# sdrobert/pydrobert-speech

Measured on AMD Instinct MI355X. Metric: frames/s (whole node) + HBM-roofline %, 40-mel fbank 16kHz 25/10ms, higher is better.
Workload: dtype f32

## Files before the change

pydrobert-speech_amd/csrc/pds_internal.h:

```cpp
#pragma once
#include <hip/hip_runtime.h>
#include <stdint.h>

#include <exception>
#include <new>
#include <string>

#include "../../include/pds_amd.h"

namespace pds {

void set_error(const std::string &msg);
int32_t hip_fail(hipError_t err, const char *what);

#define PDS_HIP(call)                                       \
  do {                                                      \
    hipError_t _e = (call);                                 \
    if (_e != hipSuccess) return pds::hip_fail(_e, #call);  \
  } while (0)

struct FastTables {
  int kind = 0;
  int n1 = 0, n2 = 0;
  int rows = 0;
  int num_cus = 0;
  float *d_window = nullptr;
  float *d_twiddle = nullptr;
  float *d_tw_special = nullptr;
  float *d_win_half = nullptr;
// ... 1 lines not shown
  float *d_ell_w = nullptr;
  int32_t *d_ell_meta = nullptr;
  int32_t *d_ell_len = nullptr;
  int32_t *d_ell_woff = nullptr;
  int ell_wfloats = 0, ell_slots = 0;
  float *d_seg_w = nullptr;
  int32_t *d_seg_meta = nullptr;
  int seg_rounds = 0, seg_len = 0, seg_wfloats = 0, seg_meta_ints = 0;
  float *d_rs_w = nullptr;
  int32_t *d_rs_meta = nullptr;
  int rs_rounds = 0, rs_len = 0, rs_wfloats = 0;
  float *d_rsn_w = nullptr;
  int32_t *d_rsn_meta = nullptr;
  int rsn_rounds = 0, rsn_len = 0, rsn_wfloats = 0;
  int rs_eslot = -1;
  float *d_ms_w = nullptr;
  int32_t *d_ms_meta = nullptr;
  int ms_rounds = 0, ms_len = 0, ms_wfloats = 0, ms_meta_ints = 0, ms_slots = 0;
  long ms_reads = 0;
  int walk = 0;
  long rs_reads = 0, rs_cost = 0, ell_reads = 0, seg_reads = 0;
  float *d_mf_tab = nullptr;
  int mf_rows = 0;
};

}

struct pds_stft_plan {
  pds_stft_desc d;
  int device = 0;
  int num_bins = 0;
  float *d_window_f32 = nullptr;
  double *d_window_f64 = nullptr;
  int32_t *d_row_ptr = nullptr;
  int32_t *d_col = nullptr;
  float *d_val_f32 = nullptr;
  double *d_val_f64 = nullptr;
  float2 *d_tw_f32 = nullptr;
  double2 *d_tw_f64 = nullptr;
  pds::FastTables fast;
};

namespace pds {
struct SiFftTables {
  int blocks = 0;
  bool big = false;
// ... 126 lines not shown
```

pydrobert-speech_amd/csrc/stft_fast.hip:

```cpp
#include "stft_wave_launch.h"

namespace pds {

#if PDS_STAMPS
unsigned long long *g_stamp_buf = nullptr;
extern "C" __attribute__((visibility("default"))) void pds_debug_set_stamp_buffer(unsigned long long *d_buf) {
  g_stamp_buf = d_buf;
}
#endif

extern "C" __attribute__((visibility("default"))) int32_t pds_build_experiments(void) { return PDS_EXPERIMENTS ? 1 : 0; }

bool fast_has_f64in(const pds_stft_plan *plan) { return plan->fast.kind && fast_f64in_kind(plan->fast.kind); }

static int fast_geometry_rows(const FastTables &ft, int *minw);

bool fast_has_fused_cmvn(const pds_stft_plan *plan) {
  const FastTables &ft = plan->fast;
  int minw = 0;
  if (!ft.kind || ft.n2 != 16 || (ft.n1 != 32 && ft.n1 != 64) || !fast_geometry_rows(ft, &minw)) return false;
  return ft.walk == 1 || ft.walk == 3 || (ft.walk == 2 && minw <= 2);
}

bool fast_has_fused_deltas(const pds_stft_plan *plan) {
  const FastTables &ft = plan->fast;
  return ft.kind && fast_deltas_kind(ft.kind) && ft.rsn_rounds >= 1 && ft.rsn_rounds <= 2 &&
         (!plan->d.include_energy || ft.rs_eslot >= 0);
}

__global__ __launch_bounds__(1024) void chunk_prefix_kernel(const int64_t *nframes, int B, int groups, int64_t *prefix) {
  __shared__ int64_t part[1024];
  const int per = (B + 1023) / 1024, lo = threadIdx.x * per, hi = lo + per < B ? lo + per : B;
  int64_t sum = 0;
  for (int b = lo; b < hi; ++b) sum += (nframes[b] + groups - 1) / groups;
// ... 168 lines not shown
    }
    ell_len[sl] = longest;
    ell_woff[sl] = (int32_t)ell_w.size();
    const int wstride = longest + 4;
    ell_w.resize(ell_w.size() + (size_t)n2 * wstride, 0.0f);
    for (int j = 0; j < n2; ++j) {
      const int f = sl * n2 + j < d.num_filts ? order[sl * n2 + j] : -1;
      if (first[j] + longest > pstr)
        first[j] = (pstr - longest) & ~3;
      if (first[j] < 0) return PDS_OK;
      ell_meta[(size_t)sl * n2 + j] = first[j] | ((f + 1) << 16);
      if (f < 0) continue;
      for (int q = row_ptr[f]; q < row_ptr[f + 1]; ++q) {
        const int t = col[q] - first[j];
        if (t < 0 || t >= longest) return PDS_OK;
        ell_w[(size_t)ell_woff[sl] + (size_t)j * wstride + t] = (float)val[q];
      }
    }
  }
  if (ell_w.empty()) ell_w.assign(4, 0.0f);
  ft.ell_wfloats = (int)ell_w.size();
  ft.ell_slots = slots;
  int32_t rc = PDS_OK;
  const int groups = 64 / n2;
  bool dense_bank = false;
  long dense_reads = 0;
  if ((n2 == 16 || (pow2 && n2 >= 32)) && d.num_filts > 0 && d.num_filts <= 65535) {
    long ell_reads = 0;
    for (int sl = 0; sl < slots; ++sl) ell_reads += 2L * (ell_len[sl] / 4);
    ft.ell_reads = ell_reads;
    const int free_slots = (wave_area_floats(n1, n2) - groups * pstr) / groups;
    int best_len = 0, best_rounds = 0;
    long best_reads = 0, any_reads = 0;
    const char *only_len = std::getenv("PDS_SEG_LEN");
    for (int len : {16, 32, 64}) {
      if (only_len && std::atoi(only_len) != len) continue;
      long nseg = 0;
      for (int f = 0; f < d.num_filts; ++f) nseg += (span(f) + len - 1) / len;
      const int rounds = (int)((nseg + 63) / 64);
      if (rounds == 0 || rounds * 64 > 65535) continue;
      int longest = 0;
      for (int f = 0; f < d.num_filts; ++f) longest = std::max(longest, (span(f) + len - 1) / len);
      const long reads = (long)rounds * (len / 4) * (1 + groups) + rounds + (nseg + 63) / 64 + 4 + 4L * ((longest + 3) / 4);
      if (!any_reads || reads < any_reads) any_reads = reads;
      if (rounds * 64 > free_slots) continue;
      if (!best_len || reads < best_reads) best_len = len, best_rounds = rounds, best_reads = reads;
// ... 19 lines not shown
        const int count = (span(f) + len - 1) / len;
        seg_meta[(size_t)nslots + f] = slot | (count << 16);
        const int base = count ? col[row_ptr[f]] & ~3 : 0;
        for (int k = 0; k < count; ++k, ++slot) {
          int first = base + k * len;
          if (first + len > pstr) first = (pstr - len) & ~3;
          if (first < 0) ok = false;
          seg_meta[slot] = first;
          for (int q = row_ptr[f]; q < row_ptr[f + 1]; ++q) {
            if (col[q] < base + k * len || col[q] >= base + (k + 1) * len) continue;
            const int t = col[q] - first;
            if (t < 0 || t >= len) ok = false; else seg_w[(size_t)slot * wstride + t] = (float)val[q];
          }
        }
      }
      if (ok) {
        ft.seg_reads = best_reads;
        ft.seg_rounds = best_rounds;
        ft.seg_len = len;
        ft.seg_wfloats = (int)seg_w.size();
        ft.seg_meta_ints = (int)seg_meta.size();
        if (rc == PDS_OK) rc = upload(&ft.d_seg_w, seg_w.data(), seg_w.size());
        if (rc == PDS_OK) rc = upload(&ft.d_seg_meta, seg_meta.data(), seg_meta.size());
      }
    }
  }
  if (n2 == 16 && rc == PDS_OK) {
    RsegTables rs;
    const int area_floats = wave_area_floats(n1, n2);
    if (build_rseg(d.num_filts, row_ptr, col, val, N / 2 + 1, area_floats / 4, 8, rs)) {
      ft.rs_rounds = rs.rounds;
      ft.rs_len = rs.seg_len;
      ft.rs_wfloats = (int)rs.w.size();
      ft.rs_reads = rs.reads_per_lane();
      ft.rs_cost = rs.cost;
      RsegTables rn;
      ft.rs_eslot = -1;
      if (rc == PDS_OK && fast_deltas_kind(N) && build_rseg(d.num_filts, row_ptr, col, val, N / 2 + 1, area_floats / 4, 2, rn, true)) {
        ft.rsn_rounds = rn.rounds;
        ft.rsn_len = rn.seg_len;
        ft.rsn_wfloats = (int)rn.w.size();
        for (size_t at = 0; at < rn.meta.size() && ft.rs_eslot < 0; ++at)
          if ((rn.meta[at] >> 16) == 0) ft.rs_eslot = (int)at;
        rc = upload(&ft.d_rsn_w, rn.w.data(), rn.w.size());
        if (rc == PDS_OK) rc = upload(&ft.d_rsn_meta, rn.meta.data(), rn.meta.size());
      }
      if (rc == PDS_OK) rc = upload(&ft.d_rs_w, rs.w.data(), rs.w.size());
      if (rc == PDS_OK) rc = upload(&ft.d_rs_meta, rs.meta.data(), rs.meta.size());
    }
  }
  if (n2 == 16 && pow2 && rc == PDS_OK && dense_bank) {
    MsegTables ms;
    const int area_floats = wave_area_floats(n1, n2);
    const int max_slots = (area_floats - 4 * pstr) / 16;
    if (build_mseg(d.num_filts, row_ptr, col, val, pstr, max_slots, ms)) {
      ft.ms_rounds = ms.rounds;
      ft.ms_slots = ms.slots;
      ft.ms_len = ms.seg_len;
      ft.ms_wfloats = (int)ms.w.size();
      ft.ms_meta_ints = (int)ms.meta.size();
      ft.ms_reads = ms.reads_per_lane();
      rc = upload(&ft.d_ms_w, ms.w.data(), ms.w.size());
      if (rc == PDS_OK) rc = upload(&ft.d_ms_meta, ms.meta.data(), ms.meta.size());
    }
  }
  {
    const char *force = std::getenv("PDS_STFT_WALK");
    ft.walk = ft.seg_rounds > 0 ? 1 : 0;
    const bool ms_stands_in = ft.walk == 0 && dense_bank && ft.ms_rounds > 0 && N >= PDS_MSEG_MIN_N;
    const long other = ft.walk == 1 ? ft.seg_reads : ms_stands_in ? dense_reads : ft.ell_reads;
    if (ft.rs_rounds > 0 && 10 * ft.rs_reads <= 7 * other) ft.walk = 2;
    if (force && std::strcmp(force, "ell") == 0) ft.walk = 0;
    if (force && std::strcmp(force, "seg") == 0) ft.walk = ft.seg_rounds > 0 ? 1 : 0;
    if (force && std::strcmp(force, "rseg") == 0) ft.walk = ft.rs_rounds > 0 ? 2 : ft.walk;
    if ((ft.walk == 1 || (ft.walk == 0 && ms_stands_in)) && ft.ms_rounds > 0 && N >= PDS_MSEG_MIN_N && !force) ft.walk = 3;
    if (force && std::strcmp(force, "mseg") == 0 && ft.ms_rounds > 0) ft.walk = 3;
    if (std::getenv("PDS_DEBUG_PLAN"))
      std::fprintf(stderr,
                   "pds plan N=%d filters=%d: ell slots %d reads %ld | seg rounds %d len %d reads %ld | rseg rounds %d "
                   "len %d reads %ld cost %ld | mseg rounds %d len %d reads %ld -> walk %d\n",
                   N, d.num_filts, ft.ell_slots, ft.ell_reads, ft.seg_rounds, ft.seg_len, ft.seg_reads, ft.rs_rounds,
                   ft.rs_len, ft.rs_reads, ft.rs_cost, ft.ms_rounds, ft.ms_len, ft.ms_reads, ft.walk);
  }
  if (rc == PDS_OK) rc = upload(&ft.d_ell_w, ell_w.data(), ell_w.size());
  if (rc == PDS_OK) rc = upload(&ft.d_ell_meta, ell_meta.data(), ell_meta.size());
  if (rc == PDS_OK) rc = upload(&ft.d_ell_len, ell_len.data(), ell_len.size());
  if (rc == PDS_OK) rc = upload(&ft.d_ell_woff, ell_woff.data(), ell_woff.size());
  if (rc == PDS_OK) rc = upload(&ft.d_window, win.data(), win.size());
  if (rc == PDS_OK) rc = upload(&ft.d_twiddle, tw.data(), tw.size());
  if (((n1 == 32 || n1 == 64) && n2 == 16) || lean_geometry(n1, n2)) {
    std::vector<float> wh(win), seed((size_t)n2 * 6);
    for (float &v : wh) v *= PDS_RDFT_DIT ? 1.0f : 0.5f;
    const int mult[3] = {1, 4, n1 / 4};
    for (int r = 0; r < n2; ++r)
      for (int j = 0; j < 3; ++j) {
        const double ang = -2.0 * M_PI * (double)((r * mult[j]) % N) / (double)N;
        seed[((size_t)r * 3 + j) * 2 + 0] = (float)std::cos(ang);
        seed[((size_t)r * 3 + j) * 2 + 1] = (float)std::sin(ang);
      }
    if (rc == PDS_OK) rc = upload(&ft.d_win_half, wh.data(), wh.size());
    if (rc == PDS_OK) rc = upload(&ft.d_tw_seed, seed.data(), seed.size());
  }
  std::vector<float> tws((size_t)n2 * 2);
  for (int r = 0; r < n2; ++r) {
    const double ang = -2.0 * M_PI * (double)r / (double)(2 * n2);
    tws[2 * r] = (float)std::cos(ang);
    tws[2 * r + 1] = (float)std::sin(ang);
  }
  if (rc == PDS_OK) rc = upload(&ft.d_tw_special, tws.data(), tws.size());
  {
    const char *front = PDS_EXPERIMENTS ? std::getenv("PDS_STFT_FRONT") : nullptr;
    const int rows = (d.frame_length + n2 - 1) / n2;
    int bucket = 0;
    for (int b : {20, 25, 28, 30, 32})
// ... 5 lines not shown
      image.reserve(mt.words());
      image.insert(image.end(), mt.win.begin(), mt.win.end());
      for (int32_t v : mt.off) {
        float f;
        std::memcpy(&f, &v, sizeof f);
        image.push_back(f);
      }
      image.insert(image.end(), mt.emask.begin(), mt.emask.end());
      image.insert(image.end(), mt.a_re.begin(), mt.a_re.end());
      image.insert(image.end(), mt.a_im.begin(), mt.a_im.end());
      image.insert(image.end(), mt.tw.begin(), mt.tw.end());
      rc = upload(&ft.d_mf_tab, image.data(), image.size());
      ft.mf_rows = bucket;
    }
  }
  if (rc != PDS_OK) return rc;
  hipDeviceProp_t prop;
  PDS_HIP(hipGetDeviceProperties(&prop, plan->device));
  ft.num_cus = prop.multiProcessorCount;
  ft.n1 = n1;
  ft.n2 = n2;
  ft.rows = (d.frame_length + n2 - 1) / n2;
  ft.kind = d.dft_size;
  return PDS_OK;
}

void fast_tables_destroy(pds_stft_plan *plan) {
  FastTables &ft = plan->fast;
  (void)hipFree(ft.d_window);
  (void)hipFree(ft.d_twiddle);
  (void)hipFree(ft.d_tw_special);
  (void)hipFree(ft.d_win_half);
  (void)hipFree(ft.d_tw_seed);
  (void)hipFree(ft.d_mf_tab);
  (void)hipFree(ft.d_rs_w);
  (void)hipFree(ft.d_ms_w);
  (void)hipFree(ft.d_ms_meta);
  (void)hipFree(ft.d_rsn_w);
  (void)hipFree(ft.d_rsn_meta);
  (void)hipFree(ft.d_rs_meta);
  (void)hipFree(ft.d_seg_w);
  (void)hipFree(ft.d_seg_meta);
  (void)hipFree(ft.d_ell_w);
  (void)hipFree(ft.d_ell_meta);
  (void)hipFree(ft.d_ell_len);
  (void)hipFree(ft.d_ell_woff);
  ft = FastTables();
}

}
```

pydrobert-speech_amd/csrc/stft_switches.h:

```cpp
#pragma once
namespace pds {

#ifndef PDS_PRIO_PACK
#define PDS_PRIO_PACK 0x103212
#endif
#if PDS_PRIO_PACK == 0xffffff
#define PDS_PHASE(i) __builtin_amdgcn_sched_barrier(0)
#else
#define PDS_PHASE(i) do { if (PDS_PRIO_PACK >= 0) __builtin_amdgcn_s_setprio(((PDS_PRIO_PACK) >> (4 * (i))) & 3); } while (0)
#endif
#ifndef PDS_ABLATE
#define PDS_ABLATE 0
#endif
#ifndef PDS_STAMPS
#define PDS_STAMPS 0
#endif
#if PDS_STAMPS
extern unsigned long long *g_stamp_buf;
#define PDS_STAMP(i, drain)                                               \
  do {                                                                    \
    if (PDS_STAMPS == 2) break;                                           \
    __builtin_amdgcn_sched_barrier(0);                                    \
    if (drain) asm volatile("s_waitcnt vmcnt(0)" ::: "memory");           \
    const unsigned long long now_ = __builtin_readcyclecounter();         \
    st_acc[i] += now_ - st_prev;                                          \
    st_prev = now_;                                                       \
    __builtin_amdgcn_sched_barrier(0);                                    \
  } while (0)
#else
#define PDS_STAMP(i, drain) do { } while (0)
#endif
#ifndef PDS_SEG_DEEP_N
#define PDS_SEG_DEEP_N 1024
#endif
#ifndef PDS_ELL_DEEP_N
#define PDS_ELL_DEEP_N 4096
#endif
#ifndef PDS_MSEG_MIN_N
#define PDS_MSEG_MIN_N 1024
#endif
#ifndef PDS_PAIR_SPLIT
#define PDS_PAIR_SPLIT 1
#endif
#ifndef PDS_N4096_MINW
#define PDS_N4096_MINW 2
#endif
#ifndef PDS_FAST_PROLOGUE
#define PDS_FAST_PROLOGUE 1
#endif
#ifndef PDS_MSEG_RED4
#define PDS_MSEG_RED4 1
#endif
#ifndef PDS_FILTER_UNROLL
#define PDS_FILTER_UNROLL 2
#endif
#ifndef PDS_EXPERIMENTS
#define PDS_EXPERIMENTS 0
#endif
#ifndef PDS_RDFT_DIT
#define PDS_RDFT_DIT (!PDS_EXPERIMENTS)
#endif
#ifndef PDS_WINDOW_CONTRACT
#define PDS_WINDOW_CONTRACT 0
#endif
#ifndef PDS_PACKED_LDS
#define PDS_PACKED_LDS 0
#endif
#ifndef PDS_WALK_DPP_FMAC
#define PDS_WALK_DPP_FMAC 1
#endif
#ifndef PDS_PREEMPH_DPP
// ... 46 lines not shown
```

pydrobert-speech_amd/csrc/stft_wave_kernel.h:

```cpp
#pragma once
#include <algorithm>
#include <atomic>
#include <cmath>
#include <cstdio>
#include <cstdlib>
#include <cstring>
#include <type_traits>
#include <vector>

#include "fft_inlane.h"
#include "mfma_front.h"
#include "rseg_tables.h"
#include "mseg_tables.h"
#include "pds_internal.h"

#include "stft_switches.h"

namespace pds {

__device__ __forceinline__ void keep_alive(float v) { asm volatile("" ::"v"(v)); }

struct FastParams {
  const void *sig;
  const int64_t *offsets, *lengths, *nframes, *row_off;
  void *out;
  int64_t out_stride;
  const float *win_lane;
  const float2 *tw_lane;
  const float2 *tw_special;
  const float *win_half;
  const float2 *tw_seed;
  const float *ell_w;
  const int32_t *ell_meta;
  const int32_t *ell_len;
  const int32_t *ell_woff;
  int ell_wfloats, ell_slots, ell_meta_pad, ell_meta_ints;
  int seg_rounds, seg_len, num_filts;
  int L, S, pad_left, include_energy, use_power, use_log;
  float log_floor, inv_L, preemph;
  double preemph_d;
  int chunks_per_utt, num_utts;
  int waves;
  int area_f;
  unsigned waves_rcp;
  int lds_ticket_off;
  int dyn;
  const float *mf_tab;
  unsigned long long *stamps;
  const int64_t *chunk_prefix;
  double *stat_part;
  int stat_c, stat_cs;
  int lds_stat_off;
// ... 42 lines not shown
}

template <int CTRL>
__device__ __forceinline__ float dpp_add(float x) {
  return x + __int_as_float(__builtin_amdgcn_update_dpp(0, __float_as_int(x), CTRL, 0xf, 0xf, false));
}

__device__ __forceinline__ void wave_sync() {
  __builtin_amdgcn_fence(__ATOMIC_RELEASE, "wavefront");
  __builtin_amdgcn_wave_barrier();
  __builtin_amdgcn_fence(__ATOMIC_ACQUIRE, "wavefront");
}

#ifndef PDS_TWOPASS
#define PDS_TWOPASS 1
#endif
#ifndef PDS_LEAN_2048
#define PDS_LEAN_2048 1
#endif
constexpr bool lean_geometry(int n1, int n2) { return PDS_LEAN_2048 && n1 == 64 && n2 == 32; }
constexpr int wave_area_floats(int n1, int n2) {
  const int cols = (n1 - 1) / 2 + 1, groups = 64 / n2, one_pass = groups * cols * (n2 + 2) * 2;
  return (PDS_TWOPASS && n1 == 64 && n2 == 16) ? 2688 : lean_geometry(n1, n2) ? groups * cols * (n2 + 4) : one_pass;
}
constexpr int win_table_stride(int rows) { return ((rows + 3) & ~3) % 8 == 4 ? ((rows + 3) & ~3) : ((rows + 3) & ~3) + 4; }

template <int N1, int N2, int NROWS>
struct WaveGeom {
  static constexpr int N = N1 * N2;
  static constexpr int NREG = (N1 - 1) / 2;
  static constexpr int COLS = NREG + 1;
  static constexpr int CPL = (COLS + N2 - 1) / N2;
  static constexpr bool FULL = COLS % N2 == 0;
  static constexpr bool DIST = N2 >= 16;
  static constexpr int GROUPS = 64 / N2;
  static constexpr int NB = N / 2 + 1;
  static constexpr int RS = N2 + 2;
  static constexpr bool TWOPASS = PDS_TWOPASS && N1 == 64 && N2 == 16;
  static constexpr bool LEAN = lean_geometry(N1, N2);
  static constexpr int RSF = N2 + 4;
  static constexpr int XROWS = TWOPASS ? N2 : COLS;
  static constexpr int EXCH_F2 = wave_area_floats(N1, N2) / 2;
  static_assert(LEAN ? GROUPS * XROWS * RSF <= EXCH_F2 * 2 : GROUPS * XROWS * RS <= EXCH_F2, "the exchange must fit the wave's area");
  static_assert(!LEAN || (CPL == 1 && N2 >= 32), "lean form: one column per lane");
  static constexpr int PSTR = ((NB + 1 + 15) / 32) * 32 + 16;
  static_assert(GROUPS * PSTR <= EXCH_F2 * 2, "P must fit over the exchange area");
// ... 43 lines not shown
  [[maybe_unused]] const bool stats_on = STATS && p.stat_part != nullptr;
  [[maybe_unused]] auto stat_add4 = [&](const int col, const float (&v)[4], const int nf) {
    double t1 = 0.0, t2 = 0.0;
#pragma unroll
    for (int q = 0; q < 4; ++q)
      if (q < nf) {
        const double d = (double)v[q];
        t1 += d;
        t2 = fma(d, d, t2);
      }
    wstat[col] += t1;
    wstat[p.stat_cs + col] += t2;
  };
  float2 *exch = reinterpret_cast<float2 *>(wbase) + g * G::XROWS * RS;
  [[maybe_unused]] float *xf = wbase + g * (G::XROWS * G::RSF);
  float *Pg = wbase + g * PSTR;
  const int nthreads = p.waves * 64;
  float2 *sw_lds = reinterpret_cast<float2 *>(smem + p.waves * p.area_f);
  int *meta_lds = reinterpret_cast<int *>(sw_lds + N2);
  float *ellw_lds = reinterpret_cast<float *>(meta_lds + p.ell_meta_pad);
  constexpr bool TWCHAIN = (PF && PDS_PF_TW == 1) || (PAIR && (N1 == 32 || N1 == 64)) || (PDS_DLT_CHAIN && DLT > 0 && N1 == 32 && N2 == 16) || G::LEAN ||
                           (N1 == 64 && N2 == 16 && (SEG == 2 || PDS_LEAN_1024));
  constexpr bool WINLDS = PF && PDS_PF_WIN == 1;
  constexpr bool WINUSE = G::LEAN || (N1 == 64 && N2 == 16 && (SEG == 2 || PDS_LEAN_1024));
  constexpr int WSTR = win_table_stride(NROWS);
  [[maybe_unused]] float *win_lds = ellw_lds + (ELL_LDS ? p.ell_wfloats : 0);
  if constexpr (WINLDS || WINUSE) {
    const float *wsrc = TWCHAIN ? p.win_half : p.win_lane;
    for (int i = threadIdx.x; i < N2 * WSTR; i += p.waves * 64) {
      const int rr = i / WSTR, k = i - rr * WSTR;
      win_lds[i] = k < NROWS ? wsrc[rr * N1 + k] : 0.0f;
    }
  }
  if (threadIdx.x < N2) sw_lds[threadIdx.x] = p.tw_special[threadIdx.x];
  constexpr bool DYN = PDS_DYN && !STRETCH && !PF;
  [[maybe_unused]] int *ticket_lds = reinterpret_cast<int *>(smem + p.lds_ticket_off);
  if constexpr (DYN) {
    if (threadIdx.x == 0) *ticket_lds = p.waves;
  }
  if constexpr (STR && G::GROUPS == 4 && (SEG != 0 || (RSG && MINW <= 2))) {
    if (p.stat_part) {
      double *z = reinterpret_cast<double *>(smem + p.lds_stat_off);
      for (int i = threadIdx.x; i < p.waves * 2 * p.stat_cs; i += p.waves * 64) z[i] = 0.0;
    }
  }
  if constexpr (RSG) {
    int4 *rec_lds = reinterpret_cast<int4 *>(meta_lds);
    for (int i = threadIdx.x; i < p.seg_rounds * 64; i += nthreads) {
      const int m = p.ell_meta[i], f = (m >> 16) - 1;
      rec_lds[i] = make_int4((m & 0x3fff) * 16, __float_as_int((m & (1 << 14)) ? 1.0f : 0.0f),
                             __float_as_int((m & (1 << 15)) ? 1.0f : 0.0f),
                             f >= 0 ? ((p.include_energy ? 1 : 0) + f) * (int)sizeof(TOUT) : -1);
    }
  } else {
    for (int i = threadIdx.x; i < p.ell_meta_pad; i += nthreads)
      meta_lds[i] = i < p.ell_meta_ints ? p.ell_meta[i] : 0;
  }
#if PDS_FAST_PROLOGUE
  static_assert((G::EXCH_F2 * 2) % 4 == 0, "wave areas are zeroed 16 bytes at a time");
  if constexpr (ELL_LDS) {
    const float4 *src4 = reinterpret_cast<const float4 *>(p.ell_w);
    float4 *dst4 = reinterpret_cast<float4 *>(ellw_lds);
    for (int i = threadIdx.x; i < (p.ell_wfloats >> 2); i += nthreads) dst4[i] = src4[i];
  }
  {
    float4 *z4 = reinterpret_cast<float4 *>(smem);
    for (int i = threadIdx.x; i < p.waves * (p.area_f / 4); i += nthreads) z4[i] = make_float4(0.0f, 0.0f, 0.0f, 0.0f);
  }
#else
  if constexpr (ELL_LDS)
    for (int i = threadIdx.x; i < p.ell_wfloats; i += nthreads) ellw_lds[i] = p.ell_w[i];
  for (int i = threadIdx.x; i < p.waves * p.area_f; i += nthreads) smem[i] = 0.0f;
#endif
  __syncthreads();

  [[maybe_unused]] float win[(MF || WINLDS || WINUSE) ? 1 : NROWS];
  [[maybe_unused]] float twr[(MF || TWCHAIN) ? 1 : COLS], twi[(MF || TWCHAIN) ? 1 : COLS];
  [[maybe_unused]] float sd[6] = {0.0f, 0.0f, 0.0f, 0.0f, 0.0f, 0.0f};
  [[maybe_unused]] float mwin[MSLOTS], mare[MF + 1], maim[MF + 1], mtwr[4], mtwi[4];
  [[maybe_unused]] unsigned moff[MSLOTS];
  if constexpr (MF > 0) {
    const float *tab = p.mf_tab;
#pragma unroll
    for (int sl = 0; sl < MSLOTS; ++sl) {
      mwin[sl] = tab[sl * 64 + lane];
      moff[sl] = (unsigned)reinterpret_cast<const int *>(tab)[(MSLOTS + sl) * 64 + lane] * 4u;
    }
#pragma unroll
    for (int t = 0; t <= MF; ++t) {
      mare[t] = tab[(3 * MSLOTS + t) * 64 + lane];
      maim[t] = tab[(3 * MSLOTS + MF + 1 + t) * 64 + lane];
    }
#pragma unroll
    for (int v = 0; v < 4; ++v) {
      const float2 t = reinterpret_cast<const float2 *>(tab + (3 * MSLOTS + 2 * (MF + 1)) * 64)[v * 64 + lane];
      mtwr[v] = t.x;
      mtwi[v] = t.y;
    }
  } else {
    if constexpr (!WINLDS && !WINUSE) {
      const float *wsrc = TWCHAIN ? p.win_half : p.win_lane;
#pragma unroll
      for (int n1 = 0; n1 < NROWS; ++n1) win[n1] = wsrc[rho * N1 + n1];
    }
    if constexpr (TWCHAIN) {
#pragma unroll
      for (int j = 0; j < 3; ++j) {
        const float2 t = p.tw_seed[rho * 3 + j];
        sd[2 * j] = t.x;
        sd[2 * j + 1] = t.y;
      }
    } else {
#pragma unroll
      for (int k1 = 1; k1 <= NREG; ++k1) {
        const float2 t = p.tw_lane[rho * COLS + k1];
        twr[k1] = t.x;
        twi[k1] = t.y;
      }
    }
  }
  [[maybe_unused]] float pfv[PF ? NROWS : 1];
  [[maybe_unused]] float wl[WINLDS ? NROWS : 1];
  [[maybe_unused]] auto read_window = [&]() {
    if constexpr (WINLDS) {
      const float4 *w4 = reinterpret_cast<const float4 *>(win_lds + rho * WSTR);
#pragma unroll
      for (int j = 0; j < (NROWS + 3) / 4; ++j) {
        const float4 w = w4[j];
        const float wv[4] = {w.x, w.y, w.z, w.w};
#pragma unroll
        for (int u = 0; u < 4; ++u)
          if (4 * j + u < NROWS) wl[4 * j + u] = wv[u];
      }
    }
  };
  read_window();
  [[maybe_unused]] bool pf_ready = false;
  [[maybe_unused]] const int pf_lane = __mul24(g, p.S) + r;
  const int L = p.L, S = p.S;
  const bool use_power = p.use_power != 0;
  const int col0 = p.include_energy ? 1 : 0;

  int b = 0;
  int wg = blockIdx.x;
#ifndef PDS_NO_XCD_MAP
  if ((gridDim.x & 7) == 0) wg = (wg & 7) * (gridDim.x >> 3) + (wg >> 3);
#endif
  int chunk = wg * p.waves + wave;
  if constexpr (!STRETCH) {
    while (chunk >= p.chunks_per_utt && b < p.num_utts) {
      chunk -= p.chunks_per_utt;
      ++b;
    }
  }
  [[maybe_unused]] int rnd = 0, rb = 0, rc = wg * p.waves;
  if constexpr (DYN) {
    while (rc >= p.chunks_per_utt && rb < p.num_utts) {
      rc -= p.chunks_per_utt;
      ++rb;
// ... 12 lines not shown
    }
    b = rb;
    chunk = rc + o;
    while (chunk >= p.chunks_per_utt && b < p.num_utts) {
      chunk -= p.chunks_per_utt;
      ++b;
    }
  };
  [[maybe_unused]] int ticket_v = 0;
  [[maybe_unused]] auto fetch_ticket = [&]() {
    if (lane == 0) ticket_v = __hip_atomic_fetch_add(ticket_lds, 1, __ATOMIC_RELAXED, __HIP_MEMORY_SCOPE_WORKGROUP);
  };
  [[maybe_unused]] auto next_item_dyn = [&](int &nfr_, int &n_, int64_t &sig_off_, int64_t &out_row_) {
    const int last_b = b;
    take_ticket(__builtin_amdgcn_readfirstlane(ticket_v));
    const int pb_ = b < p.num_utts ? b : last_b;
    nfr_ = (int)load_const(p.nframes + pb_);
    n_ = (int)load_const(p.lengths + pb_);
    sig_off_ = load_const(p.offsets + pb_);
    out_row_ = load_const(p.row_off + pb_);
  };
  int nfr = 0, n = 0;
  int64_t sig_off = 0, out_row = 0;
  if (!STRETCH && b < p.num_utts) {
    nfr = (int)load_const(p.nframes + b);
    n = (int)load_const(p.lengths + b);
    sig_off = load_const(p.offsets + b);
    out_row = load_const(p.row_off + b);
  }
  constexpr int DR = 2;
  [[maybe_unused]] int left = 0, e_lo = 0, e_hi = 0, c_last = -1;
  [[maybe_unused]] bool piece_open = false, ran = false;
  [[maybe_unused]] float Wp[DR][4], Wc[DR][4], e_keep = 0.0f;
  if constexpr (STRETCH) {
    const int gw = wg * p.waves + wave, GW = (int)gridDim.x * p.waves;
    const int total = (int)load_const(p.chunk_prefix + p.num_utts);
    const int per = total / GW, rem = total - per * GW;
    const int pos = gw * per + (gw < rem ? gw : rem);
    left = per + (gw < rem ? 1 : 0);
    int lo = 0, hi = p.num_utts;
    while (left > 0 && hi - lo > 1) {
      const int mid = (lo + hi) >> 1;
      if ((int)load_const(p.chunk_prefix + mid) <= pos) lo = mid; else hi = mid;
    }
    b = lo;
    e_lo = left > 0 ? pos - (int)load_const(p.chunk_prefix + lo) : 0;
    chunk = 0;
#pragma unroll
    for (int rd = 0; rd < DR; ++rd)
#pragma unroll
      for (int q = 0; q < 4; ++q) Wp[rd][q] = Wc[rd][q] = 0.0f;
  }
  [[maybe_unused]] auto emit_rows = [&](const int ce, const float (&nx)[DR][4]) {
    if (p.dl_debug & 2) return;
    const int C = p.dl_inner;
    const int W = (p.dl_order + 1) * C, WS = (W + 3) & ~3;
    float *stage = wbase;
    wave_sync();
#pragma unroll
    for (int rd = 0; rd < DR; ++rd) {
      if (rd >= p.seg_rounds) break;
      const int cb = reinterpret_cast<const int4 *>(meta_lds)[rd * 64 + lane].w;
      const int col = cb >= 0 ? cb >> 2 : (p.dl_eslot == rd * 64 + lane ? 0 : -1);
      const float v[12] = {Wp[rd][0], Wp[rd][1], Wp[rd][2], Wp[rd][3], Wc[rd][0], Wc[rd][1],
                           Wc[rd][2], Wc[rd][3], nx[rd][0], nx[rd][1], nx[rd][2], nx[rd][3]};
      float *mine = stage + (col >= 0 ? col : 4 * WS + lane);
      const int wrow = col >= 0 ? WS : 0, wk = col >= 0 ? C : 0;
#pragma unroll
      for (int q = 0; q < 4; ++q) {
        float d = p.dl_f1[0] * v[q + 2];
#pragma unroll
        for (int t = 1; t < 5; ++t) d = fmaf(p.dl_f1[t], v[q + 2 + t], d);
        mine[q * wrow] = v[4 + q];
        mine[q * wrow + wk] = d;
        if (p.dl_order == 2) {
// ... 1283 lines not shown
```

pydrobert-speech_amd/csrc/stft_wave_launch.h:

```cpp
#pragma once
#include "stft_wave_kernel.h"

namespace pds {


constexpr bool fast_f64in_kind(int n) { return n == 256 || n == 512 || n == 1024 || n == 2048; }

constexpr bool fast_deltas_kind(int n) { return n == 512 || n == 1024; }


template <int N1, int N2, int NROWS, int MINW>
int32_t launch_wave(const pds_stft_plan *plan, const BatchArgs &a) {
  using G = WaveGeom<N1, N2, NROWS>;
#ifndef PDS_DLT_MINW
#define PDS_DLT_MINW 3
#endif
  constexpr int DMINW = (N1 == 64 && N2 == 16) ? 2 : MINW > PDS_DLT_MINW ? PDS_DLT_MINW : MINW;
  constexpr int CU_WAVES_STFT = 4 * MINW;
  constexpr int F64_MINW = (N1 == 64 && N2 == 16) ? 2 : MINW, F64_WAVES = 4 * F64_MINW;
  const int CU_WAVES = a.dl_K > 0 ? 4 * DMINW : a.in_f64 ? F64_WAVES : CU_WAVES_STFT;
  const FastTables &ft = plan->fast;
  FastParams p;
  p.sig = a.d_signal;
  p.offsets = a.d_offsets;
// ... 130 lines not shown
  const size_t table_bytes = (size_t)p.ell_wfloats * 4;
  if (a.in_i16 && !in_lds) {
    set_error("stft_batch_i16in: not served for this plan (filter table outside LDS)");
    return PDS_ERR_INVALID;
  }
  if (pre && !in_lds) {
    if (a.in_f64 || a.out_f64 || a.dl_K > 0 || a.d_stat_part) {
      set_error("stft_batch: fused pre-emphasis with the filter table outside LDS is served for float32 samples and plain "
                "float32 features only");
      return PDS_ERR_INVALID;
    }
    return launch_stft_generic_f32(plan, a);
  }
  p.preemph = (float)a.preemph;
  p.preemph_d = a.preemph;
  p.waves = waves;
  p.mf_tab = ft.d_mf_tab;
#if PDS_STAMPS
  p.stamps = g_stamp_buf;
#else
  p.stamps = nullptr;
#endif
  p.area_f = (int)(area_bytes / 4);
  size_t smem = waves * area_bytes + fixed + (in_lds ? table_bytes : 0);
  smem = (smem + 15) & ~(size_t)15;
  p.lds_ticket_off = (int)(smem / 4);
  smem += 16;
  p.lds_stat_off = (int)(smem / 4);
  smem += (size_t)waves * stat_pw;
  p.stat_part = nullptr;
  p.stat_c = stat_c;
  p.stat_cs = stat_cs;
  p.waves_rcp = (unsigned)((0x100000000ull + (unsigned)waves - 1) / (unsigned)waves);
  {
    const char *dyn_env = std::getenv("PDS_STFT_DYN");
    p.dyn = (dyn_env && dyn_env[0] == '0') ? 0 : 1;
  }
  constexpr bool W4 = G::GROUPS == 4;
  const bool seg = SEGOK && (walk == 1 || walk == 3), rsg = W4 && walk == 2, mseg = MSG && walk == 3;
  auto kern = pre      ? (rsg ? stft_wave_kernel<N1, N2, NROWS, CU_WAVES_K, MINW, true, true, false, 0, W4>
                              : stft_wave_kernel<N1, N2, NROWS, CU_WAVES_K, MINW, true, true>)
              : rsg    ? stft_wave_kernel<N1, N2, NROWS, CU_WAVES_K, MINW, true, false, false, 0, W4>
              : mseg   ? stft_wave_kernel<N1, N2, NROWS, MS_WAVES, MS_MINW, true, false, MSG ? 2 : 0>
              : seg    ? stft_wave_kernel<N1, N2, NROWS, CU_WAVES_K, MINW, true, false, SEGOK ? 1 : 0>
              : in_lds ? stft_wave_kernel<N1, N2, NROWS, CU_WAVES_K, MINW, true, false>
                       : stft_wave_kernel<N1, N2, NROWS, CU_WAVES_K, MINW, false, false>;
// ... 182 lines not shown
```

Before: 4.094 billion.

## Prebuild a contiguous LDS image per filter walk and copy it with vec4 loads

```diff
diff --git a/pydrobert-speech_amd/csrc/lds_image.h b/pydrobert-speech_amd/csrc/lds_image.h
--- /dev/null
+++ b/pydrobert-speech_amd/csrc/lds_image.h
@@ -0,0 +1,70 @@
+#pragma once
+#include <algorithm>
+#include <cstdint>
+#include <cstring>
+#include <vector>
+
+namespace pds {
+
+enum LdsImageKind { IMG_ELL = 0, IMG_SEG = 1, IMG_RSEG = 2, IMG_MSEG = 3, IMG_RSEG_NUMBERED = 4, IMG_ELL_GLOBAL = 5, IMG_KINDS = 6 };
+
+inline int lds_meta_pad(bool rseg, int meta_ints, int uslots, int n2) {
+  return rseg ? meta_ints * 4 : (std::max(meta_ints, uslots * n2) + 3) / 4 * 4;
+}
+
+inline void rseg_record(int32_t m, bool include_energy, uint32_t out[4]) {
+  const float one = 1.0f, zero = 0.0f;
+  const int f = (m >> 16) - 1;
+  out[0] = (uint32_t)((m & 0x3fff) * 16);
+  std::memcpy(&out[1], (m & (1 << 14)) ? &one : &zero, 4);
+  std::memcpy(&out[2], (m & (1 << 15)) ? &one : &zero, 4);
+  out[3] = (uint32_t)(f >= 0 ? ((include_energy ? 1 : 0) + f) * 4 : -1);
+}
+
+struct LdsImageSpec {
+  int n2 = 0;
+  const float *tw_special = nullptr;
+  bool rseg = false;
+  bool include_energy = false;
+  const int32_t *meta = nullptr;
+  int meta_ints = 0, meta_pad = 0;
+  const float *w = nullptr;
+  int wfloats = 0;
+  const float *win = nullptr;
+  int n1 = 0, rows = 0, wstride = 0;
+};
+
+inline bool build_lds_image(const LdsImageSpec &s, std::vector<uint32_t> &img) {
+  img.clear();
+  if ((2 * s.n2) % 4 || s.meta_pad % 4 || (s.w && s.wfloats % 4) || (s.win && s.wstride % 4)) return false;
+  if (s.rseg ? s.meta_pad != s.meta_ints * 4 : s.meta_pad < s.meta_ints) return false;
+  img.resize((size_t)2 * s.n2);
+  std::memcpy(img.data(), s.tw_special, (size_t)2 * s.n2 * 4);
+  if (s.rseg) {
+    for (int i = 0; i < s.meta_ints; ++i) {
+      uint32_t rec[4];
+      rseg_record(s.meta[i], s.include_energy, rec);
+      img.insert(img.end(), rec, rec + 4);
+    }
+  } else {
+    for (int i = 0; i < s.meta_pad; ++i) img.push_back(i < s.meta_ints ? (uint32_t)s.meta[i] : 0u);
+  }
+  if (s.w) {
+    const size_t at = img.size();
+    img.resize(at + (size_t)s.wfloats);
+    std::memcpy(img.data() + at, s.w, (size_t)s.wfloats * 4);
+  }
+  if (s.win) {
+    for (int r = 0; r < s.n2; ++r)
+      for (int k = 0; k < s.wstride; ++k) {
+        const float v = k < s.rows ? s.win[(size_t)r * s.n1 + k] : 0.0f;
+        uint32_t u;
+        std::memcpy(&u, &v, 4);
+        img.push_back(u);
+      }
+  }
+  while (img.size() % 4) img.push_back(0u);
+  return true;
+}
+
+}
diff --git a/pydrobert-speech_amd/csrc/pds_internal.h b/pydrobert-speech_amd/csrc/pds_internal.h
--- a/pydrobert-speech_amd/csrc/pds_internal.h
+++ b/pydrobert-speech_amd/csrc/pds_internal.h
@@ -5,6 +5,7 @@
 #include <exception>
 #include <new>
 #include <string>
+#include <vector>
 
 #include "../../include/pds_amd.h"
 
@@ -52,6 +53,9 @@
   long rs_reads = 0, rs_cost = 0, ell_reads = 0, seg_reads = 0;
   float *d_mf_tab = nullptr;
   int mf_rows = 0;
+  float *d_lds_image[6] = {nullptr, nullptr, nullptr, nullptr, nullptr, nullptr};
+  int lds_image_vec4[6] = {0, 0, 0, 0, 0, 0};
+  std::vector<uint32_t> lds_image_host[6];
 };
 
 }
diff --git a/pydrobert-speech_amd/csrc/stft_fast.hip b/pydrobert-speech_amd/csrc/stft_fast.hip
--- a/pydrobert-speech_amd/csrc/stft_fast.hip
+++ b/pydrobert-speech_amd/csrc/stft_fast.hip
@@ -1,4 +1,5 @@
 #include "stft_wave_launch.h"
+#include "lds_image.h"
 
 namespace pds {
 
@@ -10,6 +11,14 @@
 #endif
 
 extern "C" __attribute__((visibility("default"))) int32_t pds_build_experiments(void) { return PDS_EXPERIMENTS ? 1 : 0; }
+
+extern "C" __attribute__((visibility("default"))) int64_t pds_debug_plan_lds_image(const pds_stft_plan *plan, int32_t kind,
+                                                                                    uint32_t *buf, int64_t cap) {
+  if (!plan || kind < 0 || kind >= IMG_KINDS) return -1;
+  const std::vector<uint32_t> &img = plan->fast.lds_image_host[kind];
+  if (buf && cap > 0) std::memcpy(buf, img.data(), (size_t)std::min<int64_t>(cap, (int64_t)img.size()) * 4);
+  return (int64_t)img.size();
+}
 
 bool fast_has_f64in(const pds_stft_plan *plan) { return plan->fast.kind && fast_f64in_kind(plan->fast.kind); }
 
@@ -224,6 +233,10 @@
   ft.ell_wfloats = (int)ell_w.size();
   ft.ell_slots = slots;
   int32_t rc = PDS_OK;
+  std::vector<float> seg_w_host;
+  std::vector<int32_t> seg_meta_host;
+  RsegTables rs_host, rn_host;
+  MsegTables ms_host;
   const int groups = 64 / n2;
   bool dense_bank = false;
   long dense_reads = 0;
@@ -289,6 +302,8 @@
         ft.seg_meta_ints = (int)seg_meta.size();
         if (rc == PDS_OK) rc = upload(&ft.d_seg_w, seg_w.data(), seg_w.size());
         if (rc == PDS_OK) rc = upload(&ft.d_seg_meta, seg_meta.data(), seg_meta.size());
+        seg_w_host.swap(seg_w);
+        seg_meta_host.swap(seg_meta);
       }
     }
   }
@@ -311,9 +326,11 @@
           if ((rn.meta[at] >> 16) == 0) ft.rs_eslot = (int)at;
         rc = upload(&ft.d_rsn_w, rn.w.data(), rn.w.size());
         if (rc == PDS_OK) rc = upload(&ft.d_rsn_meta, rn.meta.data(), rn.meta.size());
+        rn_host = rn;
       }
       if (rc == PDS_OK) rc = upload(&ft.d_rs_w, rs.w.data(), rs.w.size());
       if (rc == PDS_OK) rc = upload(&ft.d_rs_meta, rs.meta.data(), rs.meta.size());
+      rs_host = rs;
     }
   }
   if (n2 == 16 && pow2 && rc == PDS_OK && dense_bank) {
@@ -329,6 +346,7 @@
       ft.ms_reads = ms.reads_per_lane();
       rc = upload(&ft.d_ms_w, ms.w.data(), ms.w.size());
       if (rc == PDS_OK) rc = upload(&ft.d_ms_meta, ms.meta.data(), ms.meta.size());
+      ms_host = ms;
     }
   }
   {
@@ -355,8 +373,10 @@
   if (rc == PDS_OK) rc = upload(&ft.d_ell_woff, ell_woff.data(), ell_woff.size());
   if (rc == PDS_OK) rc = upload(&ft.d_window, win.data(), win.size());
   if (rc == PDS_OK) rc = upload(&ft.d_twiddle, tw.data(), tw.size());
+  std::vector<float> wh;
   if (((n1 == 32 || n1 == 64) && n2 == 16) || lean_geometry(n1, n2)) {
-    std::vector<float> wh(win), seed((size_t)n2 * 6);
+    std::vector<float> seed((size_t)n2 * 6);
+    wh = win;
     for (float &v : wh) v *= PDS_RDFT_DIT ? 1.0f : 0.5f;
     const int mult[3] = {1, 4, n1 / 4};
     for (int r = 0; r < n2; ++r)
@@ -408,6 +428,48 @@
   ft.n2 = n2;
   ft.rows = (d.frame_length + n2 - 1) / n2;
   ft.kind = d.dft_size;
+  const int inst_rows = fast_geometry_rows(ft);
+  for (int kind = 0; kind < IMG_KINDS && inst_rows; ++kind) {
+    LdsImageSpec s;
+    s.n2 = n2;
+    s.tw_special = tws.data();
+    s.include_energy = d.include_energy != 0;
+    const int walk = kind == IMG_RSEG_NUMBERED ? 2 : kind == IMG_ELL_GLOBAL ? 0 : kind;
+    if (kind == IMG_ELL || kind == IMG_ELL_GLOBAL) {
+      s.meta = ell_meta.data();
+      s.meta_ints = slots * n2;
+      if (kind == IMG_ELL) s.w = ell_w.data(), s.wfloats = (int)ell_w.size();
+    } else if (kind == IMG_SEG) {
+      if (!ft.seg_rounds) continue;
+      s.meta = seg_meta_host.data(), s.meta_ints = (int)seg_meta_host.size();
+      s.w = seg_w_host.data(), s.wfloats = (int)seg_w_host.size();
+    } else if (kind == IMG_MSEG) {
+      if (!ft.ms_rounds) continue;
+      s.meta = ms_host.meta.data(), s.meta_ints = (int)ms_host.meta.size();
+      s.w = ms_host.w.data(), s.wfloats = (int)ms_host.w.size();
+    } else {
+      const RsegTables &t = kind == IMG_RSEG ? rs_host : rn_host;
+      if (!(kind == IMG_RSEG ? ft.rs_rounds : ft.rsn_rounds)) continue;
+      s.rseg = true;
+      s.meta = t.meta.data(), s.meta_ints = t.rounds * 64;
+      s.w = t.w.data(), s.wfloats = (int)t.w.size();
+    }
+    s.meta_pad = lds_meta_pad(s.rseg, s.meta_ints, USLOTS, n2);
+    if (window_in_lds(n1, n2, walk == 3)) {
+      s.win = wh.data();
+      s.n1 = n1;
+      s.rows = inst_rows;
+      s.wstride = win_table_stride(inst_rows);
+    }
+    std::vector<uint32_t> &img = ft.lds_image_host[kind];
+    if (!build_lds_image(s, img)) {
+      set_error("stft plan: a table of the fused kernel does not start on 16 bytes");
+      return PDS_ERR_INVALID;
+    }
+    rc = upload(reinterpret_cast<uint32_t **>(&ft.d_lds_image[kind]), img.data(), img.size());
+    if (rc != PDS_OK) return rc;
+    ft.lds_image_vec4[kind] = (int)(img.size() / 4);
+  }
   return PDS_OK;
 }
 
@@ -431,6 +493,7 @@
   (void)hipFree(ft.d_ell_meta);
   (void)hipFree(ft.d_ell_len);
   (void)hipFree(ft.d_ell_woff);
+  for (float *img : ft.d_lds_image) (void)hipFree(img);
   ft = FastTables();
 }
 
diff --git a/pydrobert-speech_amd/csrc/stft_switches.h b/pydrobert-speech_amd/csrc/stft_switches.h
--- a/pydrobert-speech_amd/csrc/stft_switches.h
+++ b/pydrobert-speech_amd/csrc/stft_switches.h
@@ -44,9 +44,6 @@
 #endif
 #ifndef PDS_N4096_MINW
 #define PDS_N4096_MINW 2
-#endif
-#ifndef PDS_FAST_PROLOGUE
-#define PDS_FAST_PROLOGUE 1
 #endif
 #ifndef PDS_MSEG_RED4
 #define PDS_MSEG_RED4 1
diff --git a/pydrobert-speech_amd/csrc/stft_wave_kernel.h b/pydrobert-speech_amd/csrc/stft_wave_kernel.h
--- a/pydrobert-speech_amd/csrc/stft_wave_kernel.h
+++ b/pydrobert-speech_amd/csrc/stft_wave_kernel.h
@@ -28,6 +28,8 @@
   const float *win_lane;
   const float2 *tw_lane;
   const float2 *tw_special;
+  const float4 *lds_image;
+  int lds_image_vec4;
   const float *win_half;
   const float2 *tw_seed;
   const float *ell_w;
@@ -116,6 +118,9 @@
 constexpr int wave_area_floats(int n1, int n2) {
   const int cols = (n1 - 1) / 2 + 1, groups = 64 / n2, one_pass = groups * cols * (n2 + 2) * 2;
   return (PDS_TWOPASS && n1 == 64 && n2 == 16) ? 2688 : lean_geometry(n1, n2) ? groups * cols * (n2 + 4) : one_pass;
+}
+constexpr bool window_in_lds(int n1, int n2, bool mseg) {
+  return lean_geometry(n1, n2) || (n1 == 64 && n2 == 16 && (mseg || PDS_LEAN_1024));
 }
 constexpr int win_table_stride(int rows) { return ((rows + 3) & ~3) % 8 == 4 ? ((rows + 3) & ~3) : ((rows + 3) & ~3) + 4; }
 
@@ -205,103 +210,12 @@
   constexpr bool TWCHAIN = (PF && PDS_PF_TW == 1) || (PAIR && (N1 == 32 || N1 == 64)) || (PDS_DLT_CHAIN && DLT > 0 && N1 == 32 && N2 == 16) || G::LEAN ||
                            (N1 == 64 && N2 == 16 && (SEG == 2 || PDS_LEAN_1024));
   constexpr bool WINLDS = PF && PDS_PF_WIN == 1;
-  constexpr bool WINUSE = G::LEAN || (N1 == 64 && N2 == 16 && (SEG == 2 || PDS_LEAN_1024));
+  constexpr bool WINUSE = window_in_lds(N1, N2, SEG == 2);
   constexpr int WSTR = win_table_stride(NROWS);
   [[maybe_unused]] float *win_lds = ellw_lds + (ELL_LDS ? p.ell_wfloats : 0);
-  if constexpr (WINLDS || WINUSE) {
-    const float *wsrc = TWCHAIN ? p.win_half : p.win_lane;
-    for (int i = threadIdx.x; i < N2 * WSTR; i += p.waves * 64) {
-      const int rr = i / WSTR, k = i - rr * WSTR;
-      win_lds[i] = k < NROWS ? wsrc[rr * N1 + k] : 0.0f;
-    }
-  }
-  if (threadIdx.x < N2) sw_lds[threadIdx.x] = p.tw_special[threadIdx.x];
+  static_assert(!WINUSE || TWCHAIN, "the LDS window table of the plan's image is the window times 1/2");
   constexpr bool DYN = PDS_DYN && !STRETCH && !PF;
   [[maybe_unused]] int *ticket_lds = reinterpret_cast<int *>(smem + p.lds_ticket_off);
-  if constexpr (DYN) {
-    if (threadIdx.x == 0) *ticket_lds = p.waves;
-  }
-  if constexpr (STR && G::GROUPS == 4 && (SEG != 0 || (RSG && MINW <= 2))) {
-    if (p.stat_part) {
-      double *z = reinterpret_cast<double *>(smem + p.lds_stat_off);
-      for (int i = threadIdx.x; i < p.waves * 2 * p.stat_cs; i += p.waves * 64) z[i] = 0.0;
-    }
-  }
-  if constexpr (RSG) {
-    int4 *rec_lds = reinterpret_cast<int4 *>(meta_lds);
-    for (int i = threadIdx.x; i < p.seg_rounds * 64; i += nthreads) {
-      const int m = p.ell_meta[i], f = (m >> 16) - 1;
-      rec_lds[i] = make_int4((m & 0x3fff) * 16, __float_as_int((m & (1 << 14)) ? 1.0f : 0.0f),
-                             __float_as_int((m & (1 << 15)) ? 1.0f : 0.0f),
-                             f >= 0 ? ((p.include_energy ? 1 : 0) + f) * (int)sizeof(TOUT) : -1);
-    }
-  } else {
-    for (int i = threadIdx.x; i < p.ell_meta_pad; i += nthreads)
-      meta_lds[i] = i < p.ell_meta_ints ? p.ell_meta[i] : 0;
-  }
-#if PDS_FAST_PROLOGUE
-  static_assert((G::EXCH_F2 * 2) % 4 == 0, "wave areas are zeroed 16 bytes at a time");
-  if constexpr (ELL_LDS) {
-    const float4 *src4 = reinterpret_cast<const float4 *>(p.ell_w);
-    float4 *dst4 = reinterpret_cast<float4 *>(ellw_lds);
-    for (int i = threadIdx.x; i < (p.ell_wfloats >> 2); i += nthreads) dst4[i] = src4[i];
-  }
-  {
-    float4 *z4 = reinterpret_cast<float4 *>(smem);
-    for (int i = threadIdx.x; i < p.waves * (p.area_f / 4); i += nthreads) z4[i] = make_float4(0.0f, 0.0f, 0.0f, 0.0f);
-  }
-#else
-  if constexpr (ELL_LDS)
-    for (int i = threadIdx.x; i < p.ell_wfloats; i += nthreads) ellw_lds[i] = p.ell_w[i];
-  for (int i = threadIdx.x; i < p.waves * p.area_f; i += nthreads) smem[i] = 0.0f;
-#endif
-  __syncthreads();
-
-  [[maybe_unused]] float win[(MF || WINLDS || WINUSE) ? 1 : NROWS];
-  [[maybe_unused]] float twr[(MF || TWCHAIN) ? 1 : COLS], twi[(MF || TWCHAIN) ? 1 : COLS];
-  [[maybe_unused]] float sd[6] = {0.0f, 0.0f, 0.0f, 0.0f, 0.0f, 0.0f};
-  [[maybe_unused]] float mwin[MSLOTS], mare[MF + 1], maim[MF + 1], mtwr[4], mtwi[4];
-  [[maybe_unused]] unsigned moff[MSLOTS];
-  if constexpr (MF > 0) {
-    const float *tab = p.mf_tab;
-#pragma unroll
-    for (int sl = 0; sl < MSLOTS; ++sl) {
-      mwin[sl] = tab[sl * 64 + lane];
-      moff[sl] = (unsigned)reinterpret_cast<const int *>(tab)[(MSLOTS + sl) * 64 + lane] * 4u;
-    }
-#pragma unroll
-    for (int t = 0; t <= MF; ++t) {
-      mare[t] = tab[(3 * MSLOTS + t) * 64 + lane];
-      maim[t] = tab[(3 * MSLOTS + MF + 1 + t) * 64 + lane];
-    }
-#pragma unroll
-    for (int v = 0; v < 4; ++v) {
-      const float2 t = reinterpret_cast<const float2 *>(tab + (3 * MSLOTS + 2 * (MF + 1)) * 64)[v * 64 + lane];
-      mtwr[v] = t.x;
-      mtwi[v] = t.y;
-    }
-  } else {
-    if constexpr (!WINLDS && !WINUSE) {
-      const float *wsrc = TWCHAIN ? p.win_half : p.win_lane;
-#pragma unroll
-      for (int n1 = 0; n1 < NROWS; ++n1) win[n1] = wsrc[rho * N1 + n1];
-    }
-    if constexpr (TWCHAIN) {
-#pragma unroll
-      for (int j = 0; j < 3; ++j) {
-        const float2 t = p.tw_seed[rho * 3 + j];
-        sd[2 * j] = t.x;
-        sd[2 * j + 1] = t.y;
-      }
-    } else {
-#pragma unroll
-      for (int k1 = 1; k1 <= NREG; ++k1) {
-        const float2 t = p.tw_lane[rho * COLS + k1];
-        twr[k1] = t.x;
-        twi[k1] = t.y;
-      }
-    }
-  }
   [[maybe_unused]] float pfv[PF ? NROWS : 1];
   [[maybe_unused]] float wl[WINLDS ? NROWS : 1];
   [[maybe_unused]] auto read_window = [&]() {
@@ -317,7 +231,6 @@
       }
     }
   };
-  read_window();
   [[maybe_unused]] bool pf_ready = false;
   [[maybe_unused]] const int pf_lane = __mul24(g, p.S) + r;
   const int L = p.L, S = p.S;
@@ -376,19 +289,37 @@
   };
   int nfr = 0, n = 0;
   int64_t sig_off = 0, out_row = 0;
-  if (!STRETCH && b < p.num_utts) {
-    nfr = (int)load_const(p.nframes + b);
-    n = (int)load_const(p.lengths + b);
-    sig_off = load_const(p.offsets + b);
-    out_row = load_const(p.row_off + b);
+  if constexpr (!STRETCH) {
+    const int b0 = b < p.num_utts ? b : p.num_utts - 1;
+    nfr = (int)load_const(p.nframes + b0);
+    n = (int)load_const(p.lengths + b0);
+    sig_off = load_const(p.offsets + b0);
+    out_row = load_const(p.row_off + b0);
   }
+  [[maybe_unused]] int str_total = 0;
+  if constexpr (STRETCH) str_total = (int)load_const(p.chunk_prefix + p.num_utts);
+
+  const float4 *img4 = p.lds_image;
+  float4 *tab4 = reinterpret_cast<float4 *>(sw_lds);
+  const int nimg = p.lds_image_vec4;
+  auto to_lds = [&](const int i, float4 v) {
+    if constexpr (RSG && sizeof(TOUT) == 8) {
+      const int cb = __float_as_int(v.w);
+      if (i >= N2 / 2 && i < N2 / 2 + p.seg_rounds * 64 && cb >= 0) v.w = __int_as_float(2 * cb);
+    }
+    tab4[i] = v;
+  };
+  const int img_i0 = (int)threadIdx.x < nimg ? (int)threadIdx.x : nimg - 1;
+  const float4 img_v0 = img4[img_i0];
+
+  __builtin_amdgcn_sched_barrier(0);
   constexpr int DR = 2;
   [[maybe_unused]] int left = 0, e_lo = 0, e_hi = 0, c_last = -1;
   [[maybe_unused]] bool piece_open = false, ran = false;
   [[maybe_unused]] float Wp[DR][4], Wc[DR][4], e_keep = 0.0f;
   if constexpr (STRETCH) {
     const int gw = wg * p.waves + wave, GW = (int)gridDim.x * p.waves;
-    const int total = (int)load_const(p.chunk_prefix + p.num_utts);
+    const int total = str_total;
     const int per = total / GW, rem = total - per * GW;
     const int pos = gw * per + (gw < rem ? gw : rem);
     left = per + (gw < rem ? 1 : 0);
@@ -405,6 +336,77 @@
 #pragma unroll
       for (int q = 0; q < 4; ++q) Wp[rd][q] = Wc[rd][q] = 0.0f;
   }
+  static_assert((G::EXCH_F2 * 2) % 4 == 0, "wave areas are zeroed 16 bytes at a time");
+  {
+    float4 *z4 = reinterpret_cast<float4 *>(smem);
+    for (int i = threadIdx.x; i < p.waves * (p.area_f / 4); i += nthreads) z4[i] = make_float4(0.0f, 0.0f, 0.0f, 0.0f);
+  }
+  if constexpr (DYN) {
+    if (threadIdx.x == 0) *ticket_lds = p.waves;
+  }
+  if constexpr (STATS) {
+    if (p.stat_part) {
+      double *z = reinterpret_cast<double *>(smem + p.lds_stat_off);
+      for (int i = threadIdx.x; i < p.waves * 2 * p.stat_cs; i += nthreads) z[i] = 0.0;
+    }
+  }
+  if ((int)threadIdx.x < nimg) to_lds(threadIdx.x, img_v0);
+#pragma unroll 1
+  for (int i = threadIdx.x + nthreads; i < nimg; i += nthreads) to_lds(i, img4[i]);
+  if constexpr (WINLDS && !WINUSE) {
+    const float *wsrc = TWCHAIN ? p.win_half : p.win_lane;
+    for (int i = threadIdx.x; i < N2 * WSTR; i += nthreads) {
+      const int rr = i / WSTR, k = i - rr * WSTR;
+      win_lds[i] = k < NROWS ? wsrc[rr * N1 + k] : 0.0f;
+    }
+  }
+  __syncthreads();
+  [[maybe_unused]] float win[(MF || WINLDS || WINUSE) ? 1 : NROWS];
+  [[maybe_unused]] float twr[(MF || TWCHAIN) ? 1 : COLS], twi[(MF || TWCHAIN) ? 1 : COLS];
+  [[maybe_unused]] float sd[6] = {0.0f, 0.0f, 0.0f, 0.0f, 0.0f, 0.0f};
+  [[maybe_unused]] float mwin[MSLOTS], mare[MF + 1], maim[MF + 1], mtwr[4], mtwi[4];
+  [[maybe_unused]] unsigned moff[MSLOTS];
+  if constexpr (MF > 0) {
+    const float *tab = p.mf_tab;
+#pragma unroll
+    for (int sl = 0; sl < MSLOTS; ++sl) {
+      mwin[sl] = tab[sl * 64 + lane];
+      moff[sl] = (unsigned)reinterpret_cast<const int *>(tab)[(MSLOTS + sl) * 64 + lane] * 4u;
+    }
+#pragma unroll
+    for (int t = 0; t <= MF; ++t) {
+      mare[t] = tab[(3 * MSLOTS + t) * 64 + lane];
+      maim[t] = tab[(3 * MSLOTS + MF + 1 + t) * 64 + lane];
+    }
+#pragma unroll
+    for (int v = 0; v < 4; ++v) {
+      const float2 t = reinterpret_cast<const float2 *>(tab + (3 * MSLOTS + 2 * (MF + 1)) * 64)[v * 64 + lane];
+      mtwr[v] = t.x;
+      mtwi[v] = t.y;
+    }
+  } else {
+    if constexpr (!WINLDS && !WINUSE) {
+      const float *wsrc = TWCHAIN ? p.win_half : p.win_lane;
+#pragma unroll
+      for (int n1 = 0; n1 < NROWS; ++n1) win[n1] = wsrc[rho * N1 + n1];
+    }
+    if constexpr (TWCHAIN) {
+#pragma unroll
+      for (int j = 0; j < 3; ++j) {
+        const float2 t = p.tw_seed[rho * 3 + j];
+        sd[2 * j] = t.x;
+        sd[2 * j + 1] = t.y;
+      }
+    } else {
+#pragma unroll
+      for (int k1 = 1; k1 <= NREG; ++k1) {
+        const float2 t = p.tw_lane[rho * COLS + k1];
+        twr[k1] = t.x;
+        twi[k1] = t.y;
+      }
+    }
+  }
+  read_window();
   [[maybe_unused]] auto emit_rows = [&](const int ce, const float (&nx)[DR][4]) {
     if (p.dl_debug & 2) return;
     const int C = p.dl_inner;
diff --git a/pydrobert-speech_amd/csrc/stft_wave_launch.h b/pydrobert-speech_amd/csrc/stft_wave_launch.h
--- a/pydrobert-speech_amd/csrc/stft_wave_launch.h
+++ b/pydrobert-speech_amd/csrc/stft_wave_launch.h
@@ -1,5 +1,6 @@
 #pragma once
 #include "stft_wave_kernel.h"
+#include "lds_image.h"
 
 namespace pds {
 
@@ -176,6 +177,16 @@
   p.stamps = nullptr;
 #endif
   p.area_f = (int)(area_bytes / 4);
+  {
+    const int kind = !in_lds ? IMG_ELL_GLOBAL : walk == 2 ? (dl ? IMG_RSEG_NUMBERED : IMG_RSEG) : walk;
+    const size_t region = fixed - (walk == 2 && in_lds && pf_ok ? pf_extra : 0) + (in_lds ? table_bytes : 0);
+    if (!ft.d_lds_image[kind] || (size_t)ft.lds_image_vec4[kind] * 16 != region) {
+      set_error("stft_batch: the plan holds no LDS image for this launch's filter walk");
+      return PDS_ERR_INVALID;
+    }
+    p.lds_image = reinterpret_cast<const float4 *>(ft.d_lds_image[kind]);
+    p.lds_image_vec4 = ft.lds_image_vec4[kind];
+  }
   size_t smem = waves * area_bytes + fixed + (in_lds ? table_bytes : 0);
   smem = (smem + 15) & ~(size_t)15;
   p.lds_ticket_off = (int)(smem / 4);
```

Measured after the change: 4.088 billion. Within noise of the previous version (-0.2%).
